# VincentStimper/normalizing-flows

Measured on AMD Instinct MI355X. Metric: samples/sec + NLL (nats/dim), 32-layer RQ-NSF d=64 B=65536, higher is better.
Workload: dtype f32; 1 GPU; BASELINE configs[1]: log_prob of 32 x [CoupledRQS(d=64, 2 blocks, 128 hidden, K=8, tail 3) + LULinearPermute(64)] + DiagGaussian, batch 65536 rows/GPU, N(0,I) inputs, sigma=0.01 perturbed seeded weights; rows_per_gpu=65536, global_rows=65536, layers=32, launch=hipGraph replay, parallelism=dp1

## Files before the change

normalizing-flows_amd/csrc/fused_common.hpp:

```cpp
#pragma once
#include "common.hpp"

namespace nf {

constexpr int F_MAX_LAYERS = 64;

typedef float f32x16 __attribute__((ext_vector_type(16)));
typedef float f32x4 __attribute__((ext_vector_type(4)));

constexpr int F_D = 64;
constexpr int F_NI = 32;
constexpr int F_H = 128;
constexpr int F_K = 8;
constexpr int F_M = 3 * F_K - 1;
constexpr int F_STAGE = 4096;
constexpr int F_TABW = 3 * (F_K + 1);
constexpr int F_HDR = 64;

struct FusedLayout {
    int nblk;
    int K = F_K;
    __host__ __device__ int ngroups() const { return K; }
    __host__ __device__ int nfinal() const { return 3 * K; }
    __host__ __device__ int tabw() const { return 3 * (K + 1); }
// ... 251 lines not shown
    if constexpr (Z0) {
        static_assert(KB == 8, "the compact final section");
#define NF_MAX8(q, o) fmax_raw(fmax3_raw(fmax3_raw(fmax3_raw0(q[o + 1], q[o + 2]), q[o + 3], q[o + 4]), q[o + 5], q[o + 6]), q[o + 7])
        mw = f32x2e{NF_MAX8(prm0, 0), NF_MAX8(prm1, 0)};
        mh = f32x2e{NF_MAX8(prm0, KB), NF_MAX8(prm1, KB)};
#undef NF_MAX8
    } else {
#pragma unroll
        for (int k = 1; k < KB; ++k) {
            mw = f32x2e{fmaxf(mw[0], prm0[k]), fmaxf(mw[1], prm1[k])};
            mh = f32x2e{fmaxf(mh[0], prm0[KB + k]), fmaxf(mh[1], prm1[KB + k])};
        }
    }
    f32x2e pw[KB], ph[KB];
#pragma unroll
    for (int k = 0; k < KB; ++k) {
        const f32x2e aw = f32x2e{prm0[k], prm1[k]} - mw, ah = f32x2e{prm0[KB + k], prm1[KB + k]} - mh;
        const f32x2e ew = {__builtin_amdgcn_exp2f(aw[0]), __builtin_amdgcn_exp2f(aw[1])};
        const f32x2e eh = {__builtin_amdgcn_exp2f(ah[0]), __builtin_amdgcn_exp2f(ah[1])};
        pw[k] = k == 0 ? ew : pw[k - 1] + ew;
        ph[k] = k == 0 ? eh : ph[k - 1] + eh;
    }
    const f32x2e cw = ((p.right - p.left) * p.scale_w) * pk_rcp(pw[KB - 1]);
    const f32x2e ch = ((p.top - p.bottom) * p.scale_h) * pk_rcp(ph[KB - 1]);
    f32x2e kw[KB + 1], kh[KB + 1], dp[KB + 1];
    kw[0] = pk_bc(p.left);
    kh[0] = pk_bc(p.bottom);
    kw[KB] = pk_bc(p.right);
    kh[KB] = pk_bc(p.top);
    dp[0] = dp[KB] = pk_bc(p.edge_logit);
#pragma unroll
    for (int k = 1; k < KB; ++k) {
        kw[k] = pk_fma(pw[k - 1], cw, pk_bc(p.left + (p.right - p.left) * p.min_w * (float)k));
        kh[k] = pk_fma(ph[k - 1], ch, pk_bc(p.bottom + (p.top - p.bottom) * p.min_h * (float)k));
        dp[k] = f32x2e{prm0[2 * KB + k - 1], prm1[2 * KB + k - 1]};
    }
    f32x2e slo, shi, olo, ohi, dl0, dl1;
    if (!INVERSE)
        rqs_descend2<KB>(x, kw, kh, dp, slo, shi, olo, ohi, dl0, dl1);
    else
        rqs_descend2<KB>(x, kh, kw, dp, slo, shi, olo, ohi, dl0, dl1);
    const f32x2e d0 = p.min_d + f32x2e{fsoftplus<Z0>(dl0[0]), fsoftplus<Z0>(dl0[1])};
    const f32x2e d1 = p.min_d + f32x2e{fsoftplus<Z0>(dl1[0]), fsoftplus<Z0>(dl1[1])};
    f32x2e yy, ll;
    if (!INVERSE)
        rqs_eval_bin_fast2<false, Z0>(x, slo, shi - slo, olo, ohi - olo, d0, d1, yy, ll);
    else
        rqs_eval_bin_fast2<true, Z0>(x, olo, ohi - olo, slo, shi - slo, d0, d1, yy, ll);
    const f32x2e yr = inside ? yy : x;
    const f32x2e lr = inside ? ll : pk_bc(0.0f);
    y0 = yr[0]; y1 = yr[1]; lad0 = lr[0]; lad1 = lr[1];
}

template <int N>
__device__ __forceinline__ void rqs_descend1(float x, const float (&s)[N + 1], const float (&o)[N + 1], const float (&d)[N + 1],
                                             float &slo, float &shi, float &olo, float &ohi, float &dl0, float &dl1) {
    if constexpr (N == 1) {
        slo = s[0]; shi = s[1]; olo = o[0]; ohi = o[1]; dl0 = d[0]; dl1 = d[1];
    } else {
        constexpr int H = N / 2;
        const bool c = x >= s[H];
        float s2[H + 1], o2[H + 1], d2[H + 1];
#pragma unroll
        for (int i = 0; i <= H; ++i) {
            s2[i] = c ? s[H + i] : s[i];
            o2[i] = c ? o[H + i] : o[i];
            d2[i] = c ? d[H + i] : d[i];
        }
        rqs_descend1<H>(x, s2, o2, d2, slo, shi, olo, ohi, dl0, dl1);
    }
}

template <bool INVERSE, int KB = F_K>
__device__ __forceinline__ void rqs_regs_t(const RqsParams<float> &p, float x, const float (&prm)[3 * KB], float &y, float &lad) {
    static_assert((KB & (KB - 1)) == 0, "binary descent");
    const bool inside = x >= p.left && x <= p.right;
    float mw = prm[0], mh = prm[KB];
#pragma unroll
    for (int k = 1; k < KB; ++k) {
        mw = fmaxf(mw, prm[k]);
        mh = fmaxf(mh, prm[KB + k]);
    }
    float pw[KB], ph[KB];
#pragma unroll
    for (int k = 0; k < KB; ++k) {
        const float ew = __builtin_amdgcn_exp2f(prm[k] - mw), eh = __builtin_amdgcn_exp2f(prm[KB + k] - mh);
        pw[k] = k == 0 ? ew : pw[k - 1] + ew;
        ph[k] = k == 0 ? eh : ph[k - 1] + eh;
    }
    const float cw = (p.right - p.left) * p.scale_w * frcp(pw[KB - 1]);
    const float ch = (p.top - p.bottom) * p.scale_h * frcp(ph[KB - 1]);
    float kw[KB + 1], kh[KB + 1], dp[KB + 1];
    kw[0] = p.left;
    kh[0] = p.bottom;
    kw[KB] = p.right;
    kh[KB] = p.top;
    dp[0] = dp[KB] = p.edge_logit;
#pragma unroll
    for (int k = 1; k < KB; ++k) {
        kw[k] = fmaf(pw[k - 1], cw, p.left + (p.right - p.left) * p.min_w * (float)k);
        kh[k] = fmaf(ph[k - 1], ch, p.bottom + (p.top - p.bottom) * p.min_h * (float)k);
        dp[k] = prm[2 * KB + k - 1];
    }
    float slo, shi, olo, ohi, dl0, dl1;
    if (!INVERSE)
        rqs_descend1<KB>(x, kw, kh, dp, slo, shi, olo, ohi, dl0, dl1);
// ... 59 lines not shown
    }
    float slo, shi, olo, ohi, dl0, dl1;
    if (!INVERSE)
        rqs_descend1<H>(x, kw, kh, d2, slo, shi, olo, ohi, dl0, dl1);
    else
        rqs_descend1<H>(x, kh, kw, d2, slo, shi, olo, ohi, dl0, dl1);
    const float d0 = p.min_d + fsoftplus(dl0), d1 = p.min_d + fsoftplus(dl1);
    float yy, ll;
    if (!INVERSE)
        rqs_eval_bin_fast<false>(x, slo, shi - slo, olo, ohi - olo, d0, d1, yy, ll);
    else
        rqs_eval_bin_fast<true>(x, olo, ohi - olo, slo, shi - slo, d0, d1, yy, ll);
    y = inside ? yy : x;
    lad = inside ? ll : 0.0f;
}

template <bool INVERSE, int KB = F_K>
__device__ __forceinline__ void rqs_table_fast(const RqsParams<float> &p, float x, const float *tab, float &y, float &lad) {
    const bool inside = x >= p.left && x <= p.right;
    const float *srch = INVERSE ? tab + (KB + 1) : tab;
    int bin = 0;
#pragma unroll
    for (int k = 1; k < KB; ++k) bin = (x >= srch[k]) ? k : bin;
    const float cw0 = tab[bin], cw1 = tab[bin + 1], ch0 = tab[KB + 1 + bin], ch1 = tab[KB + 2 + bin];
    const float d0 = tab[2 * (KB + 1) + bin], d1 = tab[2 * (KB + 1) + bin + 1];
    float yy, ll;
    rqs_eval_bin_fast<INVERSE>(x, cw0, cw1 - cw0, ch0, ch1 - ch0, d0, d1, yy, ll);
    y = inside ? yy : x;
    lad = inside ? ll : 0.0f;
}

template <bool INVERSE, int KB = F_K>
__device__ __forceinline__ void rqs_table_fast2(const RqsParams<float> &p, float x0, float x1, const float *tab0, const float *tab1,
                                                float &y0, float &y1, float &lad0, float &lad1) {
    const f32x2e x = {x0, x1};
    const i32x2e inside = (x >= p.left) & (x <= p.right);
    const float *srch0 = INVERSE ? tab0 + (KB + 1) : tab0, *srch1 = INVERSE ? tab1 + (KB + 1) : tab1;
    int b0 = 0, b1 = 0;
#pragma unroll
    for (int k = 1; k < KB; ++k) {
        b0 = (x0 >= srch0[k]) ? k : b0;
        b1 = (x1 >= srch1[k]) ? k : b1;
    }
    const f32x2e cw0 = {tab0[b0], tab1[b1]}, cw1 = {tab0[b0 + 1], tab1[b1 + 1]};
    const f32x2e ch0 = {tab0[KB + 1 + b0], tab1[KB + 1 + b1]}, ch1 = {tab0[KB + 2 + b0], tab1[KB + 2 + b1]};
    const f32x2e d0 = {tab0[2 * (KB + 1) + b0], tab1[2 * (KB + 1) + b1]}, d1 = {tab0[2 * (KB + 1) + b0 + 1], tab1[2 * (KB + 1) + b1 + 1]};
    f32x2e yy, ll;
    rqs_eval_bin_fast2<INVERSE, false>(x, cw0, cw1 - cw0, ch0, ch1 - ch0, d0, d1, yy, ll);
    const f32x2e yr = inside ? yy : x;
    const f32x2e lr = inside ? ll : pk_bc(0.0f);
    y0 = yr[0]; y1 = yr[1]; lad0 = lr[0]; lad1 = lr[1];
}

__device__ __forceinline__ f32x16 load_bias16(const float *src) {
    const f32x4 a = *reinterpret_cast<const f32x4 *>(src), b = *reinterpret_cast<const f32x4 *>(src + 4),
                c = *reinterpret_cast<const f32x4 *>(src + 8), d = *reinterpret_cast<const f32x4 *>(src + 12);
    f32x16 v;
    v[0] = a[0]; v[1] = a[1]; v[2] = a[2]; v[3] = a[3];
    v[4] = b[0]; v[5] = b[1]; v[6] = b[2]; v[7] = b[3];
    v[8] = c[0]; v[9] = c[1]; v[10] = c[2]; v[11] = c[3];
    v[12] = d[0]; v[13] = d[1]; v[14] = d[2]; v[15] = d[3];
    return v;
}


}
```

normalizing-flows_amd/csrc/rqs_fused.hip:

```cpp
#include "fused_common.hpp"
#include <type_traits>

#define NF_TRAIN_STORE(ptr, val) __builtin_nontemporal_store((val), (ptr))

#ifdef NF_FUSED_SECONDARY
#define rqs_fused_kernel rqs_fused_kernel_nw4
#endif

namespace nf {

#ifndef NF_FUSED_SECONDARY
__global__ void pack_init_kernel(const float *__restrict__ W , const float *__restrict__ b, float *__restrict__ stage,
                                 float *__restrict__ bias_dst) {
    for (int i = blockIdx.x * blockDim.x + threadIdx.x; i < F_STAGE; i += gridDim.x * blockDim.x) {
        const int r4 = i & 3, lane = (i >> 2) & 63, s = (i >> 8) & 3, m = i >> 10;
        const int row = 32 * m + (lane & 31);
        const int k = 8 * s + 4 * (lane >> 5) + r4;
        stage[i] = W[row * F_NI + k];
    }
    for (int i = blockIdx.x * blockDim.x + threadIdx.x; i < 128; i += gridDim.x * blockDim.x) {
        const int reg = i & 15, hh = (i >> 4) & 1, m = i >> 5;
        bias_dst[i] = b[32 * m + 8 * (reg >> 2) + 4 * hh + (reg & 3)];
    }
}

__global__ void pack_hidden_kernel(const float *__restrict__ W , const float *__restrict__ b,
                                   float *__restrict__ stages , float *__restrict__ bias_dst) {
    for (int i = blockIdx.x * blockDim.x + threadIdx.x; i < 4 * F_STAGE; i += gridDim.x * blockDim.x) {
        const int r4 = i & 3, lane = (i >> 2) & 63, s = (i >> 8) & 15, m = i >> 12;
        const int row = 32 * m + (lane & 31);
        const int k = 8 * s + 4 * (lane >> 5) + r4;
        stages[i] = W[row * F_H + k];
    }
    for (int i = blockIdx.x * blockDim.x + threadIdx.x; i < 128; i += gridDim.x * blockDim.x) {
        const int reg = i & 15, hh = (i >> 4) & 1, m = i >> 5;
        bias_dst[i] = b[32 * m + 8 * (reg >> 2) + 4 * hh + (reg & 3)];
    }
}

template <int KB>
__global__ void pack_final_kernel(const float *__restrict__ W , const float *__restrict__ b,
                                  float *__restrict__ stages , float *__restrict__ bias_dst,
                                  float wh_scale) {
    constexpr int M = 3 * KB - 1;
    for (int i = blockIdx.x * blockDim.x + threadIdx.x; i < 3 * KB * F_STAGE; i += gridDim.x * blockDim.x) {
        const int r4 = i & 3, lane = (i >> 2) & 63, s = (i >> 8) & 15, st = i >> 12;
        const int g = st / 3, rb = st % 3;
        const int row = final_row_k<KB>(g, rb, lane & 31);
        const int k = 8 * s + 4 * (lane >> 5) + r4;
        const float sc = (row >= 0 && (row % M) < 2 * KB) ? wh_scale : 1.0f;
        stages[i] = row >= 0 ? W[row * F_H + k] * sc : 0.0f;
    }
    for (int i = blockIdx.x * blockDim.x + threadIdx.x; i < 96 * KB; i += gridDim.x * blockDim.x) {
        const int reg = i & 15, hh = (i >> 4) & 1, st = i >> 5;
        const int g = st / 3, rb = st % 3;
        const int row = final_row_k<KB>(g, rb, 8 * (reg >> 2) + 4 * hh + (reg & 3));
        const float sc = (row >= 0 && (row % M) < 2 * KB) ? wh_scale : 1.0f;
        bias_dst[i] = row >= 0 ? b[row] * sc : 0.0f;
    }
}

__device__ __forceinline__ void pack_compact_body(const float *__restrict__ W , const float *__restrict__ b,
                                                  float *__restrict__ stages , float *__restrict__ bias_dst,
                                                  float wh_scale, int64_t tid0, int64_t nth) {
    for (int64_t i = tid0; i < (int64_t)F_NCOMPACT * F_STAGE; i += nth) {
        const int r4 = i & 3, lane = (i >> 2) & 63, s = (i >> 8) & 15, rb = (int)(i >> 12);
        const int k = 8 * s + 4 * (lane >> 5) + r4;
        stages[i] = compact_value(rb, lane & 31, wh_scale, [=](int row) { return W[row * F_H + k]; });
    }
    for (int64_t i = tid0; i < 32 * F_NCOMPACT; i += nth) {
        const int reg = i & 15, hh = (i >> 4) & 1, rb = (int)(i >> 5);
        bias_dst[i] = compact_value(rb, 8 * (reg >> 2) + 4 * hh + (reg & 3), wh_scale, [=](int row) { return b[row]; });
    }
}
__global__ void pack_compact_kernel(const float *__restrict__ W, const float *__restrict__ b, float *__restrict__ stages,
                                    float *__restrict__ bias_dst, float wh_scale) {
    pack_compact_body(W, b, stages, bias_dst, wh_scale, (int64_t)blockIdx.x * blockDim.x + threadIdx.x, (int64_t)gridDim.x * blockDim.x);
}

__global__ void pack_tables_kernel(const float *__restrict__ uw, const float *__restrict__ uh, const float *__restrict__ ud,
                                   float *__restrict__ tab, RqsParams<float> p) {
    const int j = blockIdx.x * blockDim.x + threadIdx.x;
    if (j >= F_NI) return;
    const int K = p.K;
    const float *wj = uw + j * K, *hj = uh + j * K, *dj = ud + j * (K - 1);
    auto wacc = [=](int k) { return wj[k]; };
    auto hacc = [=](int k) { return hj[k]; };
    auto dacc = [=](int k) { return dj[k]; };
    rqs_build_table<float>(p, wacc, hacc, dacc, tab + j * 3 * (K + 1));
}

__global__ void pack_header_kernel(float *__restrict__ hdr, int nblk) {
    if (threadIdx.x == 0 && blockIdx.x == 0) {
        hdr[0] = 355.0f;
        hdr[1] = (float)nblk;
        hdr[2] = 0.0f;
        hdr[3] = 0.0f;
    }
}

__global__ void pack_final_all_kernel(const float *__restrict__ W, const float *__restrict__ b, float *__restrict__ stages,
                                      float *__restrict__ bias_dst, float wh_scale, float *__restrict__ hdr, int nblk,
                                      const float *__restrict__ uw, const float *__restrict__ uh,
                                      const float *__restrict__ ud, float *__restrict__ tab, RqsParams<float> p) {
    for (int i = blockIdx.x * blockDim.x + threadIdx.x; i < 24 * F_STAGE; i += gridDim.x * blockDim.x) {
        const int r4 = i & 3, lane = (i >> 2) & 63, s = (i >> 8) & 15, st = i >> 12;
        const int g = st / 3, rb = st % 3;
        const int row = final_row(g, rb, lane & 31);
        const int k = 8 * s + 4 * (lane >> 5) + r4;
        const float sc = (row >= 0 && (row % F_M) < 2 * F_K) ? wh_scale : 1.0f;
        stages[i] = row >= 0 ? W[row * F_H + k] * sc : 0.0f;
    }
    for (int i = blockIdx.x * blockDim.x + threadIdx.x; i < 768; i += gridDim.x * blockDim.x) {
        const int reg = i & 15, hh = (i >> 4) & 1, st = i >> 5;
        const int g = st / 3, rb = st % 3;
        const int row = final_row(g, rb, 8 * (reg >> 2) + 4 * hh + (reg & 3));
        const float sc = (row >= 0 && (row % F_M) < 2 * F_K) ? wh_scale : 1.0f;
        bias_dst[i] = row >= 0 ? b[row] * sc : 0.0f;
    }
    if (blockIdx.x != gridDim.x - 1) return;
    const int j = threadIdx.x;
    if (j == 0) {
        hdr[0] = 355.0f;
        hdr[1] = (float)nblk;
        hdr[2] = 0.0f;
        hdr[3] = 0.0f;
    }
    if (j < F_NI) {
        const float *wj = uw + j * F_K, *hj = uh + j * F_K, *dj = ud + j * (F_K - 1);
        auto wacc = [=](int k) { return wj[k]; };
// ... 278 lines not shown
    for (int Q = 0; Q < 4; ++Q) {
        f32x4 a = {0.f, 0.f, 0.f, 0.f}, b = {0.f, 0.f, 0.f, 0.f};
        if (valid) {
            const float *src = x + row * F_D + 16 * Q + 8 * hh;
            a = *reinterpret_cast<const f32x4 *>(src);
            b = *reinterpret_cast<const f32x4 *>(src + 4);
        }
#pragma unroll
        for (int c = 0; c < 4; ++c) {
            st[(8 * Q + c) * 64] = a[c];
            st[(8 * Q + 4 + c) * 64] = b[c];
        }
    }
    float ld = 0.0f;

    for (int layer = 0; layer < fa.nlayers; ++layer) {
    const float *small = small2 + (layer & 1) * small_pitch;
    const int par_t = ((fa.parity >> layer) & 1ull) ? 0 : 1;
    const int par_i = par_t ^ 1;
    const float lu_lad = LU ? fa.blob[layer][3] : 0.0f;
    if (layer > 0 || !LU || DIR == 1) {
        asm volatile("s_waitcnt vmcnt(0)" ::: "memory");
        __syncthreads();
    }
    if (LU && DIR == 0) {
        float xin[32];
#pragma unroll
        for (int c = 0; c < 32; ++c) xin[c] = st[c * 64];
        const float *buf = acquire();
        const float *bsrc = small + lay.off_bias_lu(0) + hh * 16;
        f32x16 o0 = load_bias16(bsrc), o1 = load_bias16(bsrc + 32);
        lu_mm(buf, lane, xin, o0, o1);
#pragma unroll
        for (int c = 0; c < 16; ++c) {
            st[c * 64] = o0[c];
            st[(16 + c) * 64] = o1[c];
        }
        if (hh == 0) ld += lu_lad;
    }
    if (layer + 1 < fa.nlayers) issue_small(layer + 1);

    float bx[16];
    {
        const float *tabs = small + lay.off_tables();
#pragma unroll
        for (int Q = 0; Q < 4; ++Q) {
#pragma unroll
            for (int r = 0; r < 4; r += 2) {
                const int c = 8 * Q + 2 * r + par_i;
                const int f = 8 * Q + 4 * hh + r;
                const float xi0 = st[c * 64], xi1 = st[(c + 2) * 64];
                if (DIR == 1) {
                    float y0, y1, l0, l1;
                    rqs_table_fast2<true, KB>(p, xi0, xi1, tabs + f * TABW, tabs + (f + 1) * TABW, y0, y1, l0, l1);
                    st[c * 64] = y0;
                    st[(c + 2) * 64] = y1;
                    ld += l0;
                    ld += l1;
                    bx[4 * Q + r] = y0;
                    bx[4 * Q + r + 1] = y1;
                } else {
                    bx[4 * Q + r] = xi0;
                    bx[4 * Q + r + 1] = xi1;
                }
            }
        }
        if (DIR == 1) asm volatile("" : "+v"(ld));
    }

    f32x16 H0, H1, H2, H3;
    auto store_act = [&](int t, const f32x16 &V0, const f32x16 &V1, const f32x16 &V2, const f32x16 &V3) {
        if constexpr (TRAIN == 2) {
            int l_ = lane;
            asm volatile("" : "+v"(l_));
            float *tw = small2 + small_pitch + wid * 1536;
            float *twr = tw + (l_ & 31) * 36 + 4 * (l_ >> 5);
            const int rl = l_ >> 3, cl = l_ & 7;
            const float *tww = tw + rl * 36 + 4 * cl;
            const int64_t row0 = (int64_t)blockIdx.x * F_ROWS + wid * 32 + rl;
            float *dst = act_out + ((size_t)t * (size_t)B + row0) * F_H + 4 * cl;
#pragma unroll
            for (int m = 0; m < 4; ++m) {
                const f32x16 &V = m == 0 ? V0 : (m == 1 ? V1 : (m == 2 ? V2 : V3));
#pragma unroll
                for (int q = 0; q < 4; ++q)
                    *reinterpret_cast<f32x4 *>(twr + 8 * q) = f32x4{V[4 * q], V[4 * q + 1], V[4 * q + 2], V[4 * q + 3]};
                __builtin_amdgcn_fence(__ATOMIC_RELEASE, "wavefront");
                __builtin_amdgcn_wave_barrier();
#pragma unroll
                for (int it = 0; it < 4; ++it) {
                    if (row0 + 8 * it < B)
                        NF_TRAIN_STORE(reinterpret_cast<f32x4 *>(dst + (size_t)(8 * it) * F_H + 32 * m), *reinterpret_cast<const f32x4 *>(tww + 8 * it * 36));
                }
                __builtin_amdgcn_wave_barrier();
            }
        }
    };
    auto store_xlu = [&]() {
        if constexpr (TRAIN == 2 && LU) {
            if (valid) {
#pragma unroll
                for (int Q = 0; Q < 4; ++Q) {
                    f32x4 a, b;
#pragma unroll
                    for (int c = 0; c < 4; ++c) {
                        a[c] = st[(8 * Q + c) * 64];
                        b[c] = st[(8 * Q + 4 + c) * 64];
// ... 21 lines not shown
        H1 = load_bias16(bsrc + 32);
        H2 = load_bias16(bsrc + 64);
        H3 = load_bias16(bsrc + 96);
        const float *buf = acquire();
#pragma unroll
        for (int m = 0; m < HB; ++m) {
            f32x16 &acc_m = m == 0 ? H0 : (m == 1 ? H1 : (m == 2 ? H2 : H3));
#pragma unroll
            for (int s = 0; s < 4; ++s) {
                const f32x4 a = *reinterpret_cast<const f32x4 *>(buf + (m * 4 + s) * 256 + lane * 4);
#pragma unroll
                for (int r = 0; r < 4; ++r) acc_m = MFMA(a[r], bx[4 * s + r], acc_m);
            }
        }
    }

    for (int blk = 0; blk < nblk; ++blk) {
        f32x16 T0, T1, T2, T3, R0, R1, R2, R3;
        {
            const float *bsrc = small + lay.off_bias_hidden(2 * blk) + hh * 16;
            T0 = load_bias16(bsrc);
            T1 = load_bias16(bsrc + 32);
            T2 = load_bias16(bsrc + 64);
            T3 = load_bias16(bsrc + 96);
        }
        {
            const float *buf = acquire();
            if (blk == 0) store_xlu();
            store_act(2 * blk, H0, H1, H2, H3);
            if constexpr (RAW_RELU) {
#pragma unroll
                for (int c = 0; c < 16; ++c) {
                    R0[c] = relu_raw(H0[c]);
                    R1[c] = relu_raw(H1[c]);
                    R2[c] = relu_raw(H2[c]);
                    R3[c] = relu_raw(H3[c]);
                }
                mm128<false, HB, LA>(buf, lane, T0, R0, R1, R2, R3);
            } else {
                mm128<true, HB, LA>(buf, lane, T0, H0, H1, H2, H3);
            }
        }
        if constexpr (RAW_RELU) {
            if constexpr (HB >= 2) mm128<false, HB, LA>(acquire(), lane, T1, R0, R1, R2, R3);
            if constexpr (HB == 4) {
                mm128<false, HB, LA>(acquire(), lane, T2, R0, R1, R2, R3);
                mm128<false, HB, LA>(acquire(), lane, T3, R0, R1, R2, R3);
            }
        } else {
            mm128<true, HB, LA>(acquire(), lane, T1, H0, H1, H2, H3);
            mm128<true, HB, LA>(acquire(), lane, T2, H0, H1, H2, H3);
            mm128<true, HB, LA>(acquire(), lane, T3, H0, H1, H2, H3);
        }
        {
            const float *bsrc = small + lay.off_bias_hidden(2 * blk + 1) + hh * 16;
            H0 += load_bias16(bsrc);
            H1 += load_bias16(bsrc + 32);
            H2 += load_bias16(bsrc + 64);
            H3 += load_bias16(bsrc + 96);
        }
        const float *buf2 = acquire();
        store_act(1 + 2 * blk, T0, T1, T2, T3);
#pragma unroll
        for (int c = 0; c < 16; ++c) {
            T0[c] = relu_acc(T0[c]);
            T1[c] = relu_acc(T1[c]);
            T2[c] = relu_acc(T2[c]);
            T3[c] = relu_acc(T3[c]);
        }
        mm128<false, HB, LA>(buf2, lane, H0, T0, T1, T2, T3);
        if constexpr (HB >= 2) mm128<false, HB, LA>(acquire(), lane, H1, T0, T1, T2, T3);
        if constexpr (HB == 4) {
            mm128<false, HB, LA>(acquire(), lane, H2, T0, T1, T2, T3);
            mm128<false, HB, LA>(acquire(), lane, H3, T0, T1, T2, T3);
        }
    }
    }

    float prm[FPL][MP];
    auto extract = [&](const f32x16 &A0, const f32x16 &A1, const f32x16 &A2) {
#pragma unroll
        for (int v = 0; v < 48; ++v) prm[v / MP][v % MP] = v < 16 ? A0[v] : (v < 32 ? A1[v - 16] : A2[v - 32]);
    };
    auto element = [&](int g, int f) {
        const int slot = 8 * (g / GQ) + 2 * ((g % GQ) * FPL + f) + par_t;
        const float xt = st[slot * 64];
        float yt, l;
        rqs_regs_t<DIR == 1, KB>(p, xt, prm[f], yt, l);
        st[slot * 64] = yt;
        ld += l;
    };
    auto element_pair = [&](int g) {
        if constexpr (FPL == 2) {
            const int s0 = 8 * (g / GQ) + 2 * ((g % GQ) * FPL) + par_t, s1 = s0 + 2;
            float y0, y1, l0, l1;
            rqs_regs2<DIR == 1, KB>(p, st[s0 * 64], st[s1 * 64], prm[0], prm[FPL - 1], y0, y1, l0, l1);
            st[s0 * 64] = y0;
            st[s1 * 64] = y1;
            ld += l0;
            ld += l1;
        }
    };
    auto uncond_group = [&](int g) {
        const float *tabs = small + lay.off_tables();
        if constexpr (FPL >= 2 && PAIR_TAB) {
#pragma unroll
            for (int e = 0; e < FPL; e += 2) {
                const int r = FPL * (g % GQ) + e;
                const int c = 8 * (g / GQ) + 2 * r + par_i;
                const int f = 8 * (g / GQ) + 4 * hh + r;
                float y0, y1, l0, l1;
                rqs_table_fast2<false, KB>(p, st[c * 64], st[(c + 2) * 64], tabs + f * TABW, tabs + (f + 1) * TABW, y0, y1, l0, l1);
                st[c * 64] = y0;
                st[(c + 2) * 64] = y1;
                ld += l0;
                ld += l1;
            }
        } else {
#pragma unroll
            for (int e = 0; e < FPL; ++e) {
                const int r = FPL * (g % GQ) + e;
                const int c = 8 * (g / GQ) + 2 * r + par_i;
                const int f = 8 * (g / GQ) + 4 * hh + r;
                float yi, l;
                rqs_table_fast<false, KB>(p, st[c * 64], tabs + f * TABW, yi, l);
                st[c * 64] = yi;
                ld += l;
            }
        }
    };
    if constexpr (COMPACT) {
        const float *bfin = small + lay.off_bias_compact() + hh * 16;
        f32x16 E0, E1, E2, E3;
        auto pair = [&](auto jc, const f32x16 &C, f32x16 &A0, f32x16 &A1, f32x16 &A2) __attribute__((always_inline)) {
            constexpr int J = decltype(jc)::value;
            constexpr int S0 = 42 * J, RN = (S0 + 15) / 16, RE = (S0 + 42 + 15) / 16, NNEW = RE - RN;
            static_assert(NNEW == 2 || NNEW == 3, "row-blocks per pair");
            A0 = load_bias16(bfin + RN * 32);
            A1 = load_bias16(bfin + (RN + 1) * 32);
            mm128<false, HB, LA>(acquire(), lane, A0, H0, H1, H2, H3);
            mm128<false, HB, LA>(acquire(), lane, A1, H0, H1, H2, H3);
            if constexpr (NNEW == 3) {
                A2 = load_bias16(bfin + (RN + 2) * 32);
                mm128<false, HB, LA>(acquire(), lane, A2, H0, H1, H2, H3);
            }
            auto val = [&](int slot) -> float {
                const int rb = slot >> 4, e = slot & 15;
                return rb < RN ? C[e] : (rb == RN ? A0[e] : (rb == RN + 1 ? A1[e] : A2[e]));
            };
            float p0[MP], p1[MP];
#pragma unroll
            for (int v = 0; v < MP; ++v) {
                const int c = v < KB ? v - 1 : v - 2;
                const bool zero = v == 0 || v == KB || v == MP - 1;
                p0[v] = zero ? 0.0f : val(S0 + c);
                p1[v] = zero ? 0.0f : val(S0 + 21 + c);
            }
            const int s0 = 8 * (J / 2) + 4 * (J % 2) + par_t, s1 = s0 + 2;
            float y0, y1, l0, l1;
            rqs_regs2<DIR == 1, KB, true>(p, st[s0 * 64], st[s1 * 64], p0, p1, y0, y1, l0, l1);
            st[s0 * 64] = y0;
            st[s1 * 64] = y1;
            ld += l0;
            ld += l1;
            if (DIR == 0) uncond_group(J);
        };
        pair(std::integral_constant<int, 0>{}, E0, E1, E2, E3);
        if (ngrp > 1) {
            pair(std::integral_constant<int, 1>{}, E3, E0, E1, E2);
            if (ngrp > 2) {
                pair(std::integral_constant<int, 2>{}, E2, E3, E0, E1);
                if (ngrp > 3) {
                    pair(std::integral_constant<int, 3>{}, E0, E1, E2, E3);
                    if (ngrp > 4) {
                        pair(std::integral_constant<int, 4>{}, E3, E0, E1, E2);
                        if (ngrp > 5) {
                            pair(std::integral_constant<int, 5>{}, E2, E3, E0, E1);
                            if (ngrp > 6) {
                                pair(std::integral_constant<int, 6>{}, E0, E1, E2, E3);
                                if (ngrp > 7) pair(std::integral_constant<int, 7>{}, E3, E0, E1, E2);
                            }
                        }
                    }
                }
            }
        }
    } else
    for (int g = 0; g < ngrp; ++g) {
        const float *bsrc = small + lay.off_bias_final() + (g * 3) * 32 + hh * 16;
        f32x16 A0 = load_bias16(bsrc), A1 = load_bias16(bsrc + 32), A2 = load_bias16(bsrc + 64);
        {
            const float *buf = acquire(g > 0 ? 14 : 0);
            if (g == 0) {
                if (nblk == 0) store_xlu();
                store_act(2 * nblk, H0, H1, H2, H3);
            }
            mm128<false, HB, LA>(buf, lane, A0, H0, H1, H2, H3);
        }
        mm128<false, HB, LA>(acquire(), lane, A1, H0, H1, H2, H3);
        mm128<false, HB, LA>(acquire(), lane, A2, H0, H1, H2, H3);
        extract(A0, A1, A2);
        if constexpr (TRAIN) {
            int l_ = lane;
            asm volatile("" : "+v"(l_));
            float *tw = small2 + small_pitch + wid * 1536;
            const int64_t row0 = (int64_t)blockIdx.x * F_ROWS + wid * 32;
#pragma unroll
            for (int half = 0; half < 2; ++half) {
                if ((l_ >> 5) == half) {
                    float *tr = tw + (l_ & 31) * 48;
#pragma unroll
                    for (int q = 0; q < 6; ++q) {
                        const float u_ = q < 4 ? unscale : 1.0f;
// ... 68 lines not shown
    float *wfull, *wpad;
    const int64_t *iidx;
};
__device__ __forceinline__ void pack_all_body(const PackAllArgs &a, float *__restrict__ blob, float wh_scale,
                                              const RqsParams<float> &p) {
    FusedLayout lay;
    lay.nblk = a.nblk;
    float *small = blob + F_HDR, *stages = blob + lay.off_stages();
    const int nlin = 2 * a.nblk, nst = 1 + 4 * nlin + 24;
    const int64_t tid0 = (int64_t)blockIdx.x * blockDim.x + threadIdx.x, nth = (int64_t)gridDim.x * blockDim.x;
    for (int64_t i = tid0; i < (int64_t)nst * F_STAGE; i += nth) {
        const int st = (int)(i >> 12), j = (int)(i & (F_STAGE - 1));
        const int r4 = j & 3, lane = (j >> 2) & 63;
        float v;
        if (st == 0) {
            const int s = (j >> 8) & 3, m = j >> 10;
            v = a.w_init[(32 * m + (lane & 31)) * F_NI + 8 * s + 4 * (lane >> 5) + r4];
        } else if (st <= 4 * nlin) {
            const int l = (st - 1) >> 2, m = (st - 1) & 3, s = (j >> 8) & 15;
            v = a.w_blk[l][(32 * m + (lane & 31)) * F_H + 8 * s + 4 * (lane >> 5) + r4];
        } else {
            const int f = st - 1 - 4 * nlin, g = f / 3, rb = f % 3, s = (j >> 8) & 15;
            const int row = final_row(g, rb, lane & 31);
            const float sc = (row >= 0 && (row % F_M) < 2 * F_K) ? wh_scale : 1.0f;
            v = row >= 0 ? a.w_final[row * F_H + 8 * s + 4 * (lane >> 5) + r4] * sc : 0.0f;
        }
        stages[i] = v;
    }
    if (a.wfull) {
        for (int64_t i = tid0; i < F_H * F_NI; i += nth) a.wfull[a.iidx[i & 31] * F_H + (i >> 5)] = a.w_init[i];
        for (int64_t i = tid0; i < (int64_t)24 * F_STAGE; i += nth) {
            const int st = (int)(i >> 12), j = (int)(i & (F_STAGE - 1));
            const int u4 = j & 3, lane = (j >> 2) & 63, uq = (j >> 8) & 1, vv = j >> 9;
            const int row = final_bwd_row(st / 3, 8 * (st % 3) + vv, lane >> 4);
            a.wpad[i] = row >= 0 ? a.w_final[row * F_H + 16 * (4 * uq + u4) + (lane & 15)] : 0.0f;
        }
    }
    const int nbias = 128 + 128 * nlin + 768;
    for (int64_t i = tid0; i < nbias; i += nth) {
        const int reg = i & 15, hh = (i >> 4) & 1;
        float v;
        if (i < 128 + 128 * nlin) {
            const int blk = (int)(i >> 7), m = (int)((i >> 5) & 3);
            const float *b = blk == 0 ? a.b_init : a.b_blk[blk - 1];
            v = b[32 * m + 8 * (reg >> 2) + 4 * hh + (reg & 3)];
        } else {
            const int st = (int)((i - 128 - 128 * nlin) >> 5), g = st / 3, rb = st % 3;
            const int row = final_row(g, rb, 8 * (reg >> 2) + 4 * hh + (reg & 3));
            const float sc = (row >= 0 && (row % F_M) < 2 * F_K) ? wh_scale : 1.0f;
            v = row >= 0 ? a.b_final[row] * sc : 0.0f;
        }
        small[i] = v;
    }
    pack_compact_body(a.w_final, a.b_final, stages + (size_t)lay.compact_stage(0) * F_STAGE, small + lay.off_bias_compact(), wh_scale,
                      tid0, nth);
    if (blockIdx.x == gridDim.x - 1) {
        const int j = threadIdx.x;
        if (j == 0) {
            blob[0] = 355.0f;
            blob[1] = (float)a.nblk;
            blob[2] = 0.0f;
            blob[3] = 0.0f;
        }
        if (j < F_NI) {
            const float *wj = a.uw + j * F_K, *hj = a.uh + j * F_K, *dj = a.ud + j * (F_K - 1);
            auto wacc = [=](int k) { return wj[k]; };
            auto hacc = [=](int k) { return hj[k]; };
            auto dacc = [=](int k) { return dj[k]; };
            rqs_build_table<float>(p, wacc, hacc, dacc, small + lay.off_tables() + j * F_TABW);
        }
    }
}

__global__ void pack_all_kernel(PackAllArgs a, float *__restrict__ blob, float wh_scale, RqsParams<float> p) {
    pack_all_body(a, blob, wh_scale, p);
}

__global__ void pack_all_multi_kernel(const void *const *__restrict__ table, int cols, int nblk, float wh_scale, RqsParams<float> p) {
    __shared__ PackAllArgs a;
    __shared__ float *blob;
    const void *const *row = table + (size_t)blockIdx.y * cols;
    if (threadIdx.x == 0) {
        blob = (float *)row[0];
        a.w_init = (const float *)row[1]; a.b_init = (const float *)row[2];
        a.w_final = (const float *)row[3]; a.b_final = (const float *)row[4];
        a.uw = (const float *)row[5]; a.uh = (const float *)row[6]; a.ud = (const float *)row[7];
        a.wfull = (float *)row[8]; a.wpad = (float *)row[9]; a.iidx = (const int64_t *)row[10];
        a.nblk = nblk;
        for (int l = 0; l < 2 * nblk; ++l) {
            a.w_blk[l] = (const float *)row[11 + l];
            a.b_blk[l] = (const float *)row[11 + 2 * nblk + l];
        }
    }
    __syncthreads();
    pack_all_body(a, blob, wh_scale, p);
}
#endif

}

using namespace nf;

static inline bool fused_bins_ok(int K) { return K == 4 || K == 8 || K == 16; }

template <bool LU>
static int train_fwd_launch(const void *x, void *xlu_out, void *y, void *logdet, void *cond_out, void *act_out, const FlowArgs &fa,
                            int64_t B, int hidden, int num_blocks, const RqsParams<float> &p, int acc, hipStream_t st) {
    FusedLayout lay;
// ... 137 lines not shown
    if (g < 0 || g >= K || rb < 0 || rb > 2 || rho < 0 || rho > 31) return NF_EINVAL;
    return K == 4 ? final_row_k<4>(g, rb, rho) : (K == 8 ? final_row_k<8>(g, rb, rho) : final_row_k<16>(g, rb, rho));
}

extern "C" int nf_rqs_fused_compact_row(int K, int rb, int rho) {
    if (K != 8) return NF_ENOTSUP;
    if (rb < 0 || rb >= F_NCOMPACT || rho < 0 || rho > 31) return NF_EINVAL;
    return compact_row(rb, rho);
}

extern "C" int64_t nf_rqs_fused_pack_size(int nI, int nT, int hidden, int num_blocks, int K) {
    if (nI != F_NI || nT != F_NI || hidden != F_H || !fused_bins_ok(K) || num_blocks < 0 || num_blocks > 16) return NF_ENOTSUP;
    FusedLayout lay;
    lay.nblk = num_blocks;
    lay.K = K;
    return lay.total_floats() * (int64_t)sizeof(float);
}

extern "C" int nf_rqs_fused_pack(void *wpack, const void *w_init, const void *b_init, const void *const *w_blocks,
                                 const void *const *b_blocks, const void *w_final, const void *b_final, const void *uw,
                                 const void *uh, const void *ud, int nI, int nT, int hidden, int num_blocks, int K,
                                 double tail_bound, double min_bin_width, double min_bin_height, double min_derivative,
                                 nf_stream_t stream) {
    if (nI != F_NI || nT != F_NI || hidden != F_H || !fused_bins_ok(K) || num_blocks < 0 || num_blocks > 16) return NF_ENOTSUP;
    if (!wpack || !w_init || !b_init || !w_final || !b_final || !uw || !uh || !ud) return NF_EFAULT;
    if (num_blocks > 0 && (!w_blocks || !b_blocks)) return NF_EFAULT;
    if (min_bin_width * K > 1.0 || min_bin_height * K > 1.0) return NF_EINVAL;
    hipStream_t st = (hipStream_t)stream;
    FusedLayout lay;
    lay.nblk = num_blocks;
    lay.K = K;
    float *blob = (float *)wpack;
    float *small = blob + F_HDR;
    float *stages = blob + lay.off_stages();
    hipLaunchKernelGGL(pack_header_kernel, dim3(1), dim3(64), 0, st, blob, num_blocks);
    hipLaunchKernelGGL(pack_init_kernel, dim3(16), dim3(256), 0, st, (const float *)w_init, (const float *)b_init, stages,
                       small + lay.off_bias_init());
    for (int l = 0; l < 2 * num_blocks; ++l) {
        if (!w_blocks[l] || !b_blocks[l]) return NF_EFAULT;
        hipLaunchKernelGGL(pack_hidden_kernel, dim3(64), dim3(256), 0, st, (const float *)w_blocks[l],
                           (const float *)b_blocks[l], stages + (size_t)(1 + 4 * l) * F_STAGE,
                           small + lay.off_bias_hidden(l));
    }
#define NF_PACK_FINAL(KB)                                                                                            \
    hipLaunchKernelGGL(pack_final_kernel<KB>, dim3(48 * KB), dim3(256), 0, st, (const float *)w_final,                   \
                       (const float *)b_final, stages + (size_t)(1 + 8 * num_blocks) * F_STAGE,                          \
                       small + lay.off_bias_final(), (float)(1.4426950408889634 / sqrt((double)hidden)))
    if (K == 4) NF_PACK_FINAL(4);
    else if (K == 8) NF_PACK_FINAL(8);
    else NF_PACK_FINAL(16);
#undef NF_PACK_FINAL
    if (K == 8)
        hipLaunchKernelGGL(pack_compact_kernel, dim3(21 * 16), dim3(256), 0, st, (const float *)w_final, (const float *)b_final,
                           stages + (size_t)lay.compact_stage(0) * F_STAGE, small + lay.off_bias_compact(),
                           (float)(1.4426950408889634 / sqrt((double)hidden)));
    auto p = make_rqs_params<float>(K, NF_TAILS_LINEAR, tail_bound, 0, 1, 0, 1, min_bin_width, min_bin_height,
                                    min_derivative, 1.0);
    hipLaunchKernelGGL(pack_tables_kernel, dim3(1), dim3(64), 0, st, (const float *)uw, (const float *)uh,
                       (const float *)ud, small + lay.off_tables(), p);
    NF_CHECK_LAUNCH();
    return NF_OK;
}

extern "C" int nf_rqs_fused_pack_final(void *wpack, const void *w_final, const void *b_final, const void *uw, const void *uh,
                                       const void *ud, int hidden, int num_blocks, int K, double tail_bound,
                                       double min_bin_width, double min_bin_height, double min_derivative, nf_stream_t stream) {
    if (hidden != F_H || K != F_K || num_blocks < 0 || num_blocks > 16) return NF_ENOTSUP;
    if (!wpack || !w_final || !b_final || !uw || !uh || !ud) return NF_EFAULT;
    if (min_bin_width * K > 1.0 || min_bin_height * K > 1.0) return NF_EINVAL;
    hipStream_t st = (hipStream_t)stream;
    FusedLayout lay;
    lay.nblk = num_blocks;
    float *blob = (float *)wpack;
    float *small = blob + F_HDR;
    float *stages = blob + lay.off_stages();
    auto p = make_rqs_params<float>(K, NF_TAILS_LINEAR, tail_bound, 0, 1, 0, 1, min_bin_width, min_bin_height,
                                    min_derivative, 1.0);
    hipLaunchKernelGGL(pack_final_all_kernel, dim3(384), dim3(256), 0, st, (const float *)w_final, (const float *)b_final,
                       stages + (size_t)(1 + 8 * num_blocks) * F_STAGE, small + lay.off_bias_final(),
                       (float)(1.4426950408889634 / sqrt((double)hidden)), blob, num_blocks, (const float *)uw,
                       (const float *)uh, (const float *)ud, small + lay.off_tables(), p);
    NF_CHECK_LAUNCH();
    return NF_OK;
}

extern "C" int nf_rqs_fused_pack_lu(void *wpack, int num_blocks, const int64_t *perm, const void *lower_entries,
                                    const void *upper_entries, const void *unconstrained_upper_diag, const void *bias,
                                    int D, double eps, int K, nf_stream_t stream) {
    if (D != F_D || num_blocks < 0 || num_blocks > 16 || !fused_bins_ok(K)) return NF_ENOTSUP;
    if (!wpack || !perm || !lower_entries || !upper_entries || !unconstrained_upper_diag || !bias) return NF_EFAULT;
    hipStream_t st = (hipStream_t)stream;
    FusedLayout lay;
    lay.nblk = num_blocks;
    lay.K = K;
    float *blob = (float *)wpack;
    float *small = blob + F_HDR;
    float *stages = blob + lay.off_stages();
    const size_t lds = (size_t)4 * F_D * F_D * sizeof(double) + F_D * sizeof(int) + F_D * sizeof(double) + 64;
    static LdsOptIn opted = {};
    if (opt_in_lds(reinterpret_cast<const void *>(&pack_lu_kernel), lds, opted) != NF_OK) return NF_ENOTSUP;
    hipLaunchKernelGGL(pack_lu_kernel, dim3(1), dim3(256), lds, st, perm, (const float *)lower_entries,
                       (const float *)upper_entries, (const float *)unconstrained_upper_diag, (const float *)bias,
                       (float)eps, stages + (size_t)lay.lu_stage(0) * F_STAGE, stages + (size_t)lay.lu_stage(1) * F_STAGE,
                       small + lay.off_bias_lu(0), small + lay.off_bias_lu(1), blob);
    NF_CHECK_LAUNCH();
    return NF_OK;
// ... 139 lines not shown
```

Measured before the change: 13.07 million samples/s.

## Fold last hidden bias into compact final bias, specialize compact RQS path

The last residual block's second bias is folded into the compact final-layer bias at pack time (computing b_final + W_final·b2 in double), so the kernel skips the bias add for that block in the compact path. This relies on the output being linear in that bias, which assumes no nonlinearity between the bias add and the final projection. A specialized rqs_regs2_c evaluates the spline from the raw 21 logits, using max-subtracted exp2 and cumulative sums with packed ops. Table-based bin lookup switches from a linear 7-compare scan to a 3-step binary search for the compact path.

Measured after the change: 13.15 million samples/s (median of 6 runs). Within noise of the previous version (+0.5%).

```diff
diff --git a/normalizing-flows_amd/csrc/fused_common.hpp b/normalizing-flows_amd/csrc/fused_common.hpp
--- a/normalizing-flows_amd/csrc/fused_common.hpp
+++ b/normalizing-flows_amd/csrc/fused_common.hpp
@@ -327,6 +327,78 @@
     y0 = yr[0]; y1 = yr[1]; lad0 = lr[0]; lad1 = lr[1];
 }
 
+template <bool INVERSE>
+__device__ __forceinline__ void rqs_regs2_c(const RqsParams<float> &p, float x0, float x1, const float (&v0)[21], const float (&v1)[21],
+                                            float &y0, float &y1, float &lad0, float &lad1) {
+    constexpr int KB = 8;
+    const f32x2e x = {x0, x1};
+    const i32x2e inside = (x >= p.left) & (x <= p.right);
+#define NF_MAX7(q, o) fmax_raw(fmax3_raw(fmax3_raw(fmax3_raw0(q[o], q[o + 1]), q[o + 2], q[o + 3]), q[o + 4], q[o + 5]), q[o + 6])
+    const float mw0 = NF_MAX7(v0, 0), mw1 = NF_MAX7(v1, 0), mh0 = NF_MAX7(v0, 7), mh1 = NF_MAX7(v1, 7);
+#undef NF_MAX7
+    float a0[14], a1[14];
+#pragma unroll
+    for (int c = 0; c < 14; c += 2) {
+        const f32x2e d = f32x2e{v0[c], v0[c + 1]} - f32x2e{c < 7 ? mw0 : mh0, c + 1 < 7 ? mw0 : mh0};
+        a0[c] = d[0];
+        a0[c + 1] = d[1];
+    }
+    a1[0] = v1[0] - mw1;
+#pragma unroll
+    for (int c = 1; c < 13; c += 2) {
+        const f32x2e d = f32x2e{v1[c], v1[c + 1]} - pk_bc(c < 7 ? mw1 : mh1);
+        a1[c] = d[0];
+        a1[c + 1] = d[1];
+    }
+    a1[13] = v1[13] - mh1;
+    const f32x2e mw = {mw0, mw1}, mh = {mh0, mh1};
+    f32x2e pw[KB], ph[KB];
+#pragma unroll
+    for (int k = 0; k < KB; ++k) {
+        f32x2e aw, ah;
+        if (k == 0) {
+            aw = pk_bc(0.0f) - mw;
+            ah = pk_bc(0.0f) - mh;
+        } else {
+            aw = f32x2e{a0[k - 1], a1[k - 1]};
+            ah = f32x2e{a0[6 + k], a1[6 + k]};
+        }
+        const f32x2e ew = {__builtin_amdgcn_exp2f(aw[0]), __builtin_amdgcn_exp2f(aw[1])};
+        const f32x2e eh = {__builtin_amdgcn_exp2f(ah[0]), __builtin_amdgcn_exp2f(ah[1])};
+        pw[k] = k == 0 ? ew : pw[k - 1] + ew;
+        ph[k] = k == 0 ? eh : ph[k - 1] + eh;
+    }
+    const f32x2e cw = ((p.right - p.left) * p.scale_w) * pk_rcp(pw[KB - 1]);
+    const f32x2e ch = ((p.top - p.bottom) * p.scale_h) * pk_rcp(ph[KB - 1]);
+    f32x2e kw[KB + 1], kh[KB + 1], dp[KB + 1];
+    kw[0] = pk_bc(p.left);
+    kh[0] = pk_bc(p.bottom);
+    kw[KB] = pk_bc(p.right);
+    kh[KB] = pk_bc(p.top);
+    dp[0] = dp[KB] = pk_bc(p.edge_logit);
+#pragma unroll
+    for (int k = 1; k < KB; ++k) {
+        kw[k] = pk_fma(pw[k - 1], cw, pk_bc(p.left + (p.right - p.left) * p.min_w * (float)k));
+        kh[k] = pk_fma(ph[k - 1], ch, pk_bc(p.bottom + (p.top - p.bottom) * p.min_h * (float)k));
+        dp[k] = f32x2e{v0[13 + k], v1[13 + k]};
+    }
+    f32x2e slo, shi, olo, ohi, dl0, dl1;
+    if (!INVERSE)
+        rqs_descend2<KB>(x, kw, kh, dp, slo, shi, olo, ohi, dl0, dl1);
+    else
+        rqs_descend2<KB>(x, kh, kw, dp, slo, shi, olo, ohi, dl0, dl1);
+    const f32x2e d0 = p.min_d + f32x2e{fsoftplus<true>(dl0[0]), fsoftplus<true>(dl0[1])};
+    const f32x2e d1 = p.min_d + f32x2e{fsoftplus<true>(dl1[0]), fsoftplus<true>(dl1[1])};
+    f32x2e yy, ll;
+    if (!INVERSE)
+        rqs_eval_bin_fast2<false, true>(x, slo, shi - slo, olo, ohi - olo, d0, d1, yy, ll);
+    else
+        rqs_eval_bin_fast2<true, true>(x, olo, ohi - olo, slo, shi - slo, d0, d1, yy, ll);
+    const f32x2e yr = inside ? yy : x;
+    const f32x2e lr = inside ? ll : pk_bc(0.0f);
+    y0 = yr[0]; y1 = yr[1]; lad0 = lr[0]; lad1 = lr[1];
+}
+
 template <int N>
 __device__ __forceinline__ void rqs_descend1(float x, const float (&s)[N + 1], const float (&o)[N + 1], const float (&d)[N + 1],
                                              float &slo, float &shi, float &olo, float &ohi, float &dl0, float &dl1) {
@@ -492,6 +564,28 @@
     y0 = yr[0]; y1 = yr[1]; lad0 = lr[0]; lad1 = lr[1];
 }
 
+template <bool INVERSE>
+__device__ __forceinline__ void rqs_table_bin2(const RqsParams<float> &p, float x0, float x1, const float *tab0, const float *tab1,
+                                               float &y0, float &y1, float &lad0, float &lad1) {
+    constexpr int KB = 8;
+    const f32x2e x = {x0, x1};
+    const i32x2e inside = (x >= p.left) & (x <= p.right);
+    const float *srch0 = INVERSE ? tab0 + (KB + 1) : tab0, *srch1 = INVERSE ? tab1 + (KB + 1) : tab1;
+    int b0 = (x0 >= srch0[4]) ? 4 : 0, b1 = (x1 >= srch1[4]) ? 4 : 0;
+    b0 += (x0 >= srch0[b0 + 2]) ? 2 : 0;
+    b1 += (x1 >= srch1[b1 + 2]) ? 2 : 0;
+    b0 += (x0 >= srch0[b0 + 1]) ? 1 : 0;
+    b1 += (x1 >= srch1[b1 + 1]) ? 1 : 0;
+    const f32x2e cw0 = {tab0[b0], tab1[b1]}, cw1 = {tab0[b0 + 1], tab1[b1 + 1]};
+    const f32x2e ch0 = {tab0[KB + 1 + b0], tab1[KB + 1 + b1]}, ch1 = {tab0[KB + 2 + b0], tab1[KB + 2 + b1]};
+    const f32x2e d0 = {tab0[2 * (KB + 1) + b0], tab1[2 * (KB + 1) + b1]}, d1 = {tab0[2 * (KB + 1) + b0 + 1], tab1[2 * (KB + 1) + b1 + 1]};
+    f32x2e yy, ll;
+    rqs_eval_bin_fast2<INVERSE, false>(x, cw0, cw1 - cw0, ch0, ch1 - ch0, d0, d1, yy, ll);
+    const f32x2e yr = inside ? yy : x;
+    const f32x2e lr = inside ? ll : pk_bc(0.0f);
+    y0 = yr[0]; y1 = yr[1]; lad0 = lr[0]; lad1 = lr[1];
+}
+
 __device__ __forceinline__ f32x16 load_bias16(const float *src) {
     const f32x4 a = *reinterpret_cast<const f32x4 *>(src), b = *reinterpret_cast<const f32x4 *>(src + 4),
                 c = *reinterpret_cast<const f32x4 *>(src + 8), d = *reinterpret_cast<const f32x4 *>(src + 12);
diff --git a/normalizing-flows_amd/csrc/rqs_fused.hip b/normalizing-flows_amd/csrc/rqs_fused.hip
--- a/normalizing-flows_amd/csrc/rqs_fused.hip
+++ b/normalizing-flows_amd/csrc/rqs_fused.hip
@@ -61,8 +61,8 @@
 }
 
 __device__ __forceinline__ void pack_compact_body(const float *__restrict__ W , const float *__restrict__ b,
-                                                  float *__restrict__ stages , float *__restrict__ bias_dst,
-                                                  float wh_scale, int64_t tid0, int64_t nth) {
+                                                  const float *__restrict__ b2 , float *__restrict__ stages ,
+                                                  float *__restrict__ bias_dst, float wh_scale, int64_t tid0, int64_t nth) {
     for (int64_t i = tid0; i < (int64_t)F_NCOMPACT * F_STAGE; i += nth) {
         const int r4 = i & 3, lane = (i >> 2) & 63, s = (i >> 8) & 15, rb = (int)(i >> 12);
         const int k = 8 * s + 4 * (lane >> 5) + r4;
@@ -70,12 +70,22 @@
     }
     for (int64_t i = tid0; i < 32 * F_NCOMPACT; i += nth) {
         const int reg = i & 15, hh = (i >> 4) & 1, rb = (int)(i >> 5);
-        bias_dst[i] = compact_value(rb, 8 * (reg >> 2) + 4 * hh + (reg & 3), wh_scale, [=](int row) { return b[row]; });
-    }
-}
-__global__ void pack_compact_kernel(const float *__restrict__ W, const float *__restrict__ b, float *__restrict__ stages,
-                                    float *__restrict__ bias_dst, float wh_scale) {
-    pack_compact_body(W, b, stages, bias_dst, wh_scale, (int64_t)blockIdx.x * blockDim.x + threadIdx.x, (int64_t)gridDim.x * blockDim.x);
+        const int rho = 8 * (reg >> 2) + 4 * hh + (reg & 3);
+        if (b2) {
+            bias_dst[i] = compact_value(rb, rho, wh_scale, [=](int row) {
+                double a = (double)b[row];
+                for (int k = 0; k < F_H; ++k) a += (double)W[row * F_H + k] * (double)b2[k];
+                return a;
+            });
+        } else {
+            bias_dst[i] = compact_value(rb, rho, wh_scale, [=](int row) { return b[row]; });
+        }
+    }
+}
+__global__ void pack_compact_kernel(const float *__restrict__ W, const float *__restrict__ b, const float *__restrict__ b2,
+                                    float *__restrict__ stages, float *__restrict__ bias_dst, float wh_scale) {
+    pack_compact_body(W, b, b2, stages, bias_dst, wh_scale, (int64_t)blockIdx.x * blockDim.x + threadIdx.x,
+                      (int64_t)gridDim.x * blockDim.x);
 }
 
 __global__ void pack_tables_kernel(const float *__restrict__ uw, const float *__restrict__ uh, const float *__restrict__ ud,
@@ -460,7 +470,8 @@
                 const float xi0 = st[c * 64], xi1 = st[(c + 2) * 64];
                 if (DIR == 1) {
                     float y0, y1, l0, l1;
-                    rqs_table_fast2<true, KB>(p, xi0, xi1, tabs + f * TABW, tabs + (f + 1) * TABW, y0, y1, l0, l1);
+                    if constexpr (COMPACT) rqs_table_bin2<true>(p, xi0, xi1, tabs + f * TABW, tabs + (f + 1) * TABW, y0, y1, l0, l1);
+                    else rqs_table_fast2<true, KB>(p, xi0, xi1, tabs + f * TABW, tabs + (f + 1) * TABW, y0, y1, l0, l1);
                     st[c * 64] = y0;
                     st[(c + 2) * 64] = y1;
                     ld += l0;
@@ -588,7 +599,7 @@
             mm128<true, HB, LA>(acquire(), lane, T2, H0, H1, H2, H3);
             mm128<true, HB, LA>(acquire(), lane, T3, H0, H1, H2, H3);
         }
-        {
+        if (!(COMPACT && blk == nblk - 1)) {
             const float *bsrc = small + lay.off_bias_hidden(2 * blk + 1) + hh * 16;
             H0 += load_bias16(bsrc);
             H1 += load_bias16(bsrc + 32);
@@ -646,7 +657,8 @@
                 const int c = 8 * (g / GQ) + 2 * r + par_i;
                 const int f = 8 * (g / GQ) + 4 * hh + r;
                 float y0, y1, l0, l1;
-                rqs_table_fast2<false, KB>(p, st[c * 64], st[(c + 2) * 64], tabs + f * TABW, tabs + (f + 1) * TABW, y0, y1, l0, l1);
+                if constexpr (COMPACT) rqs_table_bin2<false>(p, st[c * 64], st[(c + 2) * 64], tabs + f * TABW, tabs + (f + 1) * TABW, y0, y1, l0, l1);
+                else rqs_table_fast2<false, KB>(p, st[c * 64], st[(c + 2) * 64], tabs + f * TABW, tabs + (f + 1) * TABW, y0, y1, l0, l1);
                 st[c * 64] = y0;
                 st[(c + 2) * 64] = y1;
                 ld += l0;
@@ -684,17 +696,15 @@
                 const int rb = slot >> 4, e = slot & 15;
                 return rb < RN ? C[e] : (rb == RN ? A0[e] : (rb == RN + 1 ? A1[e] : A2[e]));
             };
-            float p0[MP], p1[MP];
-#pragma unroll
-            for (int v = 0; v < MP; ++v) {
-                const int c = v < KB ? v - 1 : v - 2;
-                const bool zero = v == 0 || v == KB || v == MP - 1;
-                p0[v] = zero ? 0.0f : val(S0 + c);
-                p1[v] = zero ? 0.0f : val(S0 + 21 + c);
+            float v0[21], v1[21];
+#pragma unroll
+            for (int c = 0; c < 21; ++c) {
+                v0[c] = val(S0 + c);
+                v1[c] = val(S0 + 21 + c);
             }
             const int s0 = 8 * (J / 2) + 4 * (J % 2) + par_t, s1 = s0 + 2;
             float y0, y1, l0, l1;
-            rqs_regs2<DIR == 1, KB, true>(p, st[s0 * 64], st[s1 * 64], p0, p1, y0, y1, l0, l1);
+            rqs_regs2_c<DIR == 1>(p, st[s0 * 64], st[s1 * 64], v0, v1, y0, y1, l0, l1);
             st[s0 * 64] = y0;
             st[s1 * 64] = y1;
             ld += l0;
@@ -869,8 +879,8 @@
         }
         small[i] = v;
     }
-    pack_compact_body(a.w_final, a.b_final, stages + (size_t)lay.compact_stage(0) * F_STAGE, small + lay.off_bias_compact(), wh_scale,
-                      tid0, nth);
+    pack_compact_body(a.w_final, a.b_final, a.nblk > 0 ? a.b_blk[2 * a.nblk - 1] : nullptr,
+                      stages + (size_t)lay.compact_stage(0) * F_STAGE, small + lay.off_bias_compact(), wh_scale, tid0, nth);
     if (blockIdx.x == gridDim.x - 1) {
         const int j = threadIdx.x;
         if (j == 0) {
@@ -1114,6 +1124,7 @@
 #undef NF_PACK_FINAL
     if (K == 8)
         hipLaunchKernelGGL(pack_compact_kernel, dim3(21 * 16), dim3(256), 0, st, (const float *)w_final, (const float *)b_final,
+                           num_blocks > 0 ? (const float *)b_blocks[2 * num_blocks - 1] : (const float *)nullptr,
                            stages + (size_t)lay.compact_stage(0) * F_STAGE, small + lay.off_bias_compact(),
                            (float)(1.4426950408889634 / sqrt((double)hidden)));
     auto p = make_rqs_params<float>(K, NF_TAILS_LINEAR, tail_bound, 0, 1, 0, 1, min_bin_width, min_bin_height,
```
